# MingXiangL/SPE

Hardware: AMD Instinct MI355X
Metric: images/sec (whole node) at 3x800x1333 bs=2/GPU (higher is better)
Workload: dtype bf16/fp16 operands, fp32 accumulate; 1 GPU; TSCAM_cait_S24 (C=384, depth 24, 8 heads) + 0-layer encoder + 6-layer conditional-DETR decoder x2 stages, 100 queries, COCO heads (91), 2x3x800x1333 per GPU (N=4150 tokens), fwd + SetCriterion + SetCriterionRefine + bwd + grad all-reduce + clip + AdamW; global_batch=2, parallelism=dp1

## Files before the change

### include/spe_hip.h

```cpp
#ifndef SPE_HIP_H
#define SPE_HIP_H
#include <stddef.h>
#include <stdint.h>

#ifdef __cplusplus
extern "C" {
#endif

typedef struct ihipStream_t* spe_stream_t;

int spe_abi_version(void);

int spe_set_reduce_workspace(void* ws, size_t bytes, spe_stream_t stream);
int spe_reduce_defer_ranges(const void* const* ptrs, const size_t* bytes, int n);
int spe_reduce_defer_arena(void* arena, size_t bytes);
int spe_reduce_flush(spe_stream_t stream);
int spe_reduce_pending(void);

int spe_gemm_f32(const float* A, const float* B, float* C, const float* bias, float* C2,
                 int M, int N, int K, long lda, long ldb, long ldc, int transA, int transB,
                 int batch0, int batch1, long sA0, long sA1, long sB0, long sB1, long sC0, long sC1,
                 float alpha, int act, int splitk, int precision, spe_stream_t stream);

int spe_gemm_ex(const void* A, int a_bf16, const float* B, float* C, const float* bias, float* C2,
// ... 117 lines not shown
                          float* mean, float* rstd, long R, int C, float eps, float p, uint64_t seed, uint64_t offset,
                          spe_stream_t stream);
int spe_layernorm_res_bwd(const float* dy, const float* dy2, const float* sum, const float* gamma, const float* mean, const float* rstd,
                          float* ds, float* dz, float* dgamma, float* dbeta, long R, int C, float p, uint64_t seed,
                          uint64_t offset, spe_stream_t stream);

int spe_dropout(const float* x, float* y, long n, float p, uint64_t seed, uint64_t offset, spe_stream_t stream);

int spe_patchify(const float* img, float* cols, int B, int Cin, int Hi, int Wi, int P, spe_stream_t stream);

int spe_rowdot(const float* x, const float* y, float* D, int B, int L, int H, int dh, spe_stream_t stream);

int spe_add_rows(const float* a, const float* b, float* out, long n, long period, spe_stream_t stream);

int spe_bicubic(const float* src, float* dst, int gh, int gw, int h, int w, int C, int backward, spe_stream_t stream);

int spe_matcher_cost(const float* logits, const float* boxes, const int* tgt_ids, const float* tgt_boxes,
                     const int* toff, int total_targets, float* cost, int* err, int L, int B, int Q, int Kc,
                     float w_class, float w_bbox, float w_giou, spe_stream_t stream);

int spe_hungarian(const float* cost, const int* toff, long* srow, long* gidx, int* lidx, int* err, int L, int B, int Q,
                  spe_stream_t stream);
int spe_jitter_pick(const float* box, const float* scale, float* out, int M, int ncand, int ratio, spe_stream_t stream);

int spe_focal_loss(const float* logits, const int* tclass, const float* roww, float* grad, float* loss,
                   int* argmax, int L, long rows_per_l, int Kc, float alpha, float gamma, spe_stream_t stream);

int spe_box_loss(const float* pred_boxes, const long* srow, const float* tbox, const float* w, const int* lidx,
                 float* sums, float* g_l1, float* g_giou, long n, int L, spe_stream_t stream);
int spe_box_loss_bwd(const long* srow, const int* lidx, const float* g_l1, const float* g_giou, const float* c1,
                     const float* c2, float* dpred, long n, spe_stream_t stream);

int spe_kv_frags(const void* ym16, long ldm, const void* yp16, long ldp, void* Kf, void* V16, void* K16, void* Vf,
                 int L, int B, int S, int H, int dh, spe_stream_t stream);
int spe_kv_grad_scatter(const float* dk, const float* dv, void* dYm, long ldm, void* dYp, long ldp, int layer, int B, int S,
                        int H, int dh, spe_stream_t stream);
int spe_colsum_bf16_blocks(const void* x, long ld, long R, int nblk, int blkC, float* const* outs, int accumulate, spe_stream_t stream);

int spe_mha_plan(int B, int H, int Lq, int Lk, int* nch);
int spe_mha_fwd(const void* Qf, const void* Kf, const void* V16, const void* mask, float* Opart, float* ML, float* O,
                float* LSE, void* keepbits, int B, int H, int Lq, int Lk, int dk, int dv, int nch, float p_drop,
                uint64_t seed, uint64_t offset, spe_stream_t stream);
int spe_mha_bwd(const void* Qf, const void* Kf, const void* Vf, const void* dOf, const void* K16, const void* Q16,
                const void* dO16, const void* mask, const float* LSE, const float* D, const void* keepbits, float* dq,
                float* dq_ws, float* dk, float* dv, int B, int H, int Lq, int Lk, int dk_dim, int dv_dim, int nch, float scale,
                float p_drop, spe_stream_t stream);

int spe_pos_sine(const void* mask_u8, const float* dim_t, float* out, int B, int h, int w, int npf, float scale,
                 float eps, int normalize, spe_stream_t stream);

int spe_pos_learned_fwd(const float* col, const float* row, float* out, int B, int h, int w, int npf, spe_stream_t stream);
int spe_pos_learned_bwd(const float* g, float* d_col, float* d_row, int B, int h, int w, int npf, spe_stream_t stream);

int spe_nms_sorted(const float* boxes, const long* labels, const int* counts, unsigned char* keep, int nimg, int nmax,
                   float iou_threshold, spe_stream_t stream);

int spe_detect(const float* logits, const float* boxes, const float* sizes, int B, int Q, int Kc, int k, float iou_threshold,
               int do_nms, float* out_logit, long* out_label, float* out_box, int* out_query, int* out_count, spe_stream_t stream);

int spe_cam_prepare(const float* cams, int M, int h, int w, int rows, int cols, float cam_thr, float* minmax,
                    void* out, spe_stream_t stream);
int spe_cam_contour_boxes(const void* img, int rows, int cols, float area_ratio, int* boxes, int max_boxes, int* nboxes);
int spe_cam_boxes_device_workspace(int M, int rows, int cols, size_t* bytes);
int spe_cam_boxes_device(const void* img, int M, int rows, int cols, float area_ratio, void* workspace, size_t workspace_bytes,
                         int* boxes, int* nboxes, int max_boxes, spe_stream_t stream);

int spe_voc_match(const float* det_boxes, const float* det_scores, const long* det_labels, const int* det_off,
                  const double* gt_boxes, const long* gt_labels, const unsigned char* gt_difficult, const int* gt_off,
                  int nimg, int num_classes, int max_det, int max_gt, double ovthresh, double score_scale, double coord_scale,
                  unsigned char* flags, double* scores_out, int* npos, int* nimgs, int* hits, spe_stream_t stream);
int spe_voc_ap(const unsigned char* flags, const int* seg_off, const int* npos, int num_classes, double* ap07, double* ap_area,
               double* rec, double* prec, spe_stream_t stream);

int spe_coco_match(const float* det_boxes, const long* det_cats, const int* det_off, const double* gt_boxes, const long* gt_cats,
                   const unsigned char* gt_iscrowd, const double* gt_area, const int* gt_off, const double* iou_thrs,
                   const double* area_rng, int nimg, int num_cats, int max_det, int max_gt, int top, int* rank, unsigned* words,
                   int* npig, spe_stream_t stream);
int spe_coco_accumulate(const unsigned* words, const int* rank, const float* det_scores, const int* seg_off, const int* npig,
                        const int* max_dets, const double* rec_thrs, int num_cats, int num_rec, int num_max_dets, double* precision,
                        double* recall, double* scores, spe_stream_t stream);

int spe_resample_plan(long* desc_host, int n, long* totals);
int spe_resample_tables(const long* desc_host, const long* desc_dev, int n, int* tables, spe_stream_t stream);
int spe_resample_h(const long* desc_host, const long* desc_dev, int n, const int* tables, unsigned char* tmp, spe_stream_t stream);
int spe_resample_v(const long* desc_host, const long* desc_dev, int n, const int* tables, const unsigned char* tmp, const float* lut,
                   float* out, unsigned char* mask, int Hmax, int Wmax, spe_stream_t stream);

int spe_ledger_state_bytes(int K, int E, size_t* bytes);
int spe_ledger_record(const float* vals, const float* weights, const unsigned char* mask, const double* extras_host, int K, int E,
                      void* state, size_t state_bytes, float* total, spe_stream_t stream);
int spe_ledger_total_bwd(const float* g, const float* weights, const unsigned char* mask, int K, float* dvals, spe_stream_t stream);
int spe_ledger_summary(void* state, size_t state_bytes, int K, int E, const int* windows_host, const int* windows_dev,
                       const float* ring_override, const int* order, double* out, spe_stream_t stream);

int spe_sqnorm_partials(const float* g, long n, float* partials, int nblocks, spe_stream_t stream);
int spe_adamw_flat(float* p, float* g, float* m, float* v, long n, const long* seg_end, const float* seg_lr,
                   const float* seg_wd, int nseg, float beta1, float beta2, float eps, float bias_c1, float bias_c2,
                   const float* partials, int npartials, float max_norm, int write_grad, float grad_scale,
                   spe_stream_t stream);

int spe_accum_flat(float* dst, const float* a, const float* b, long n, spe_stream_t stream);

int spe_occupy(int nwg, long micros, float* buf, long buf_floats, spe_stream_t stream);

#ifdef __cplusplus
}
// ... 3 lines not shown
```

### spe_amd/build.py

```python
import glob
import hashlib
import os
import subprocess
import sys
from concurrent.futures import ThreadPoolExecutor

HERE = os.path.dirname(os.path.abspath(__file__))
CSRC = os.path.join(HERE, "csrc")
OBJ = os.path.join(HERE, "build")
LIB = os.path.join(HERE, "libspe_hip.so")
COMM_LIB = os.path.join(HERE, "libspe_comm.so")
STAMP = os.path.join(HERE, "libspe_hip.srchash")
FLAGS = ["--offload-arch=gfx950", "-O3", "-std=c++17", "-fPIC"]
EXTRA_FLAGS = {"attn_flash_bwd.hip": ["-mllvm", "-amdgpu-mfma-vgpr-form=1"],
               "voc_eval.hip": ["-ffp-contract=off"],
               "coco_eval.hip": ["-ffp-contract=off"],
               "img_resample.hip": ["-ffp-contract=off"],
               "step_ledger.hip": ["-ffp-contract=off"],
               "detect.hip": ["-ffp-contract=off"]}


def flags_for(src):
    return FLAGS + EXTRA_FLAGS.get(os.path.basename(src), [])


def sources():
    return sorted(glob.glob(os.path.join(CSRC, "*.hip")))


def _headers():
    return sorted(glob.glob(os.path.join(CSRC, "*.h")))


def _hash(files, extra=b""):
    h = hashlib.sha256(extra)
    for f in files:
        h.update(os.path.basename(f).encode())
        with open(f, "rb") as fh:
            h.update(fh.read())
    return h.hexdigest()


def _comm_sources():
    return sorted(glob.glob(os.path.join(CSRC, "comm", "*.hip"))) + [os.path.join(os.path.dirname(HERE), "include", "spe_comm.h")]


def source_hash():
    return _hash(sources() + _headers() + _comm_sources())


def needs_build():
    if not (os.path.exists(LIB) and os.path.exists(STAMP)):
        return True
    with open(STAMP) as fh:
        return fh.read().strip() != source_hash()


def _compile(src, hipcc, verbose):
    name = os.path.splitext(os.path.basename(src))[0]
    obj, tag = os.path.join(OBJ, name + ".o"), os.path.join(OBJ, name + ".hash")
    want = _hash([src] + _headers(), " ".join(flags_for(src)).encode())
    if os.path.exists(obj) and os.path.exists(tag) and open(tag).read().strip() == want:
        return obj
    cmd = [hipcc] + flags_for(src) + ["-c", src, "-o", obj + ".tmp"]
    if verbose:
        print(" ".join(cmd), file=sys.stderr, flush=True)
    subprocess.run(cmd, check=True, cwd=CSRC)
    os.replace(obj + ".tmp", obj)
    with open(tag, "w") as fh:
        fh.write(want + "\n")
    return obj

# ... 37 lines not shown
```

### spe_amd/kernels.py

```python
import ctypes
import os

import torch

from . import lib

_PRECISION = 2
import functools as _functools
import threading as _threading

_TLS = _threading.local()


def _in_bwd():
    return getattr(_TLS, "in_bwd", False)


def backward_scope(fn):
    @_functools.wraps(fn)
    def wrapped(ctx, *grads):
        prev, _TLS.in_bwd = _in_bwd(), True
        if _DEFER_FLATS is not None and not _FLUSH_QUEUED[0]:
            _FLUSH_QUEUED[0] = True
            try:
# ... 1406 lines not shown
    M, rows, cols = t.shape
    out = torch.empty((M * (1 + 4 * max_boxes),), device=t.device, dtype=torch.int32)
    if M:
        nbytes = cam_boxes_workspace_bytes(M, rows, cols)
        ws = torch.empty((nbytes // 4,), device=t.device, dtype=torch.int32)
        _call("spe_cam_boxes_device", _p(t), M, rows, cols, float(area_ratio), _p(ws), nbytes, _p(out[M:]), _p(out), max_boxes, _st())
    return out


def cam_boxes_device(imgs_u8_device, area_ratio, max_boxes=256):
    M = imgs_u8_device.shape[0]
    out = cam_boxes_device_packed(imgs_u8_device, area_ratio, max_boxes)
    return out[M:].view(M, max_boxes, 4), out[:M]


def pos_sine(mask_bool, dim_t, npf, scale, eps, normalize):
    B, h, w = mask_bool.shape
    m8 = mask_bool.to(torch.uint8).contiguous()
    out = torch.empty((B, h, w, 2 * npf), device=mask_bool.device, dtype=torch.float32)
    _call("spe_pos_sine", _p(m8), _p(dim_t), _p(out), B, h, w, npf, float(scale), float(eps), int(bool(normalize)), _st())
    return out


POS_TABLE_ROWS = 50


def pos_learned_fwd(col, row, B, h, w):
    _chk(col, row)
    npf = col.shape[1]
    if col.shape != (POS_TABLE_ROWS, npf) or row.shape != col.shape or not (col.is_contiguous() and row.is_contiguous()):
        raise ValueError(f"pos_learned_fwd: two contiguous [{POS_TABLE_ROWS}, npf] tables expected, got {tuple(col.shape)} and {tuple(row.shape)}")
    out = torch.empty((B, h, w, 2 * npf), device=col.device, dtype=torch.float32)
    _call("spe_pos_learned_fwd", _p(col), _p(row), _p(out), B, h, w, npf, _st())
    return out


def pos_learned_bwd(g, B, h, w, npf, need_col=True, need_row=True, dcol_out=None, drow_out=None):
    _chk(g, dcol_out, drow_out)
    if g.numel() != B * h * w * 2 * npf or not g.is_contiguous():
        raise ValueError(f"pos_learned_bwd: a contiguous gradient of {B} x {h} x {w} x {2 * npf} elements expected, got {tuple(g.shape)}")
    outs = []
    for need, o in ((need_col, dcol_out), (need_row, drow_out)):
        if not need:
            o = None
        elif o is None:
            o = torch.empty((POS_TABLE_ROWS, npf), device=g.device, dtype=torch.float32)
        elif o.shape != (POS_TABLE_ROWS, npf) or not o.is_contiguous():
            raise ValueError(f"pos_learned_bwd: destination {tuple(o.shape)} is not a contiguous [{POS_TABLE_ROWS}, {npf}]")
        outs.append(o)
    _call("spe_pos_learned_bwd", _p(g), _p(outs[0]), _p(outs[1]), B, h, w, npf, _st())
    return outs[0], outs[1]


MAX_DET = 4096
VOC_MAX_DET = COCO_MAX_DET = MAX_DET


def _check_typed(name, pairs):
    for t, dt in pairs:
        if not t.is_cuda:
            raise lib.SpeLibraryError("spe_amd kernels run on the GPU only (got a CPU tensor); there is no CPU fallback")
        if t.dtype != dt or not t.is_contiguous():
            raise TypeError(f"{name}: expected a contiguous {dt} tensor, got {t.dtype}")


VOC_MAX_GT = 1024


def voc_match(det_boxes, det_scores, det_labels, det_off, gt_boxes, gt_labels, gt_difficult, gt_off, max_det, max_gt,
              ovthresh, score_scale, coord_scale, npos, nimgs, hits):
    _check_typed("voc_match", ((det_boxes, torch.float32), (det_scores, torch.float32), (det_labels, torch.int64), (det_off, torch.int32),
                               (gt_boxes, torch.float64), (gt_labels, torch.int64), (gt_difficult, torch.uint8), (gt_off, torch.int32),
                               (npos, torch.int32), (nimgs, torch.int32), (hits, torch.int32)))
    nd, C, nimg = det_scores.numel(), npos.numel(), det_off.numel() - 1
    if gt_off.numel() != nimg + 1 or nimgs.numel() != C or hits.numel() != C or det_boxes.numel() != nd * 4 or \
            det_labels.numel() != nd or gt_boxes.numel() != gt_labels.numel() * 4 or gt_difficult.numel() != gt_labels.numel():
        raise ValueError("voc_match: inconsistent shapes")
    flags = torch.empty((nd,), device=det_scores.device, dtype=torch.uint8)
    scores = torch.empty((nd,), device=det_scores.device, dtype=torch.float64)
    _call("spe_voc_match", _p(det_boxes), _p(det_scores), _p(det_labels), _p(det_off), _p(gt_boxes), _p(gt_labels), _p(gt_difficult),
          _p(gt_off), nimg, C, int(max_det), int(max_gt), float(ovthresh), float(score_scale), float(coord_scale), _p(flags),
          _p(scores), _p(npos), _p(nimgs), _p(hits), _st())
    return flags, scores


def voc_ap(flags, seg_off, npos, want_curve=False):
    _check_typed("voc_ap", ((flags, torch.uint8), (seg_off, torch.int32), (npos, torch.int32)))
    C = npos.numel()
    if seg_off.numel() != C + 1:
        raise ValueError("voc_ap: seg_off must hold num_classes + 1 offsets")
    ap = torch.empty((2, C), device=flags.device, dtype=torch.float64)
    rec = torch.empty((flags.numel(),), device=flags.device, dtype=torch.float64) if want_curve else None
    prec = torch.empty_like(rec) if want_curve else None
    _call("spe_voc_ap", _p(flags), _p(seg_off), _p(npos), C, _p(ap[0]), _p(ap[1]), _p(rec), _p(prec), _st())
    return ap[0], ap[1], rec, prec


COCO_MAX_GT = 512
COCO_T, COCO_A = 10, 4
COCO_MAX_REC = 128


def coco_match(det_boxes, det_cats, det_off, gt_boxes, gt_cats, gt_iscrowd, gt_area, gt_off, iou_thrs, area_rng, max_det, max_gt,
               top, npig):
    _check_typed("coco_match", ((det_boxes, torch.float32), (det_cats, torch.int64), (det_off, torch.int32), (gt_boxes, torch.float64),
                                (gt_cats, torch.int64), (gt_iscrowd, torch.uint8), (gt_area, torch.float64), (gt_off, torch.int32),
# ... 114 lines not shown
```

### spe_amd/models/conditional_detr.py

```python
import math

import torch
import torch.nn.functional as F
from torch import nn
from torch.autograd import Function

from .. import kernels as K
from ..util import box_ops
from ..util.misc import (NestedTensor, get_world_size, host_to_device, inverse_sigmoid, is_dist_avail_and_initialized,
                         nested_tensor_from_tensor_list)
from .cait_backbone import build_backbone
from .layers import MLP, Linear
from .matcher import build_matcher
from .transformer import build_transformer


class ConditionalDETR_Refine(nn.Module):

    def __init__(self, backbone, transformer, num_classes, num_queries, aux_loss=False, num_refines=1, drloc=False):
        super().__init__()
        self.num_queries = num_queries
        self.num_refines = num_refines
        self.transformer = transformer
        hidden_dim = transformer.d_model
        self.class_embed = nn.ModuleList([Linear(hidden_dim, num_classes) for _ in range(num_refines + 1)])
        self.bbox_embed = nn.ModuleList([MLP(hidden_dim, hidden_dim, 4, 3) for _ in range(num_refines + 1)])
        self.query_embed = nn.Embedding(num_queries, hidden_dim)
        self.queries_embed_refine = nn.ModuleList([nn.Embedding(num_queries, hidden_dim) for _ in range(num_refines)])
        self.backbone = backbone
        self.aux_loss = aux_loss
        bias_value = -math.log((1 - 0.01) / 0.01)
        for ce in self.class_embed:
            ce.bias.data = torch.ones(num_classes) * bias_value
        for be in self.bbox_embed:
            nn.init.constant_(be.layers[-1].weight.data, 0)
            nn.init.constant_(be.layers[-1].bias.data, 0)

    def forward(self, samples: NestedTensor):
        if isinstance(samples, (list, torch.Tensor)):
            samples = nested_tensor_from_tensor_list(samples)
        _, _, H, W = samples.decompose()[0].size()
        ps = self.backbone[0].body.patch_size
        self.transformer.H, self.transformer.W = H // ps, W // ps
        features, pos = self.backbone(samples)
        src, mask = features["x_patch"].decompose()
        assert mask is not None
        Hs, references = self.transformer(src, mask, self.query_embed.weight, pos[-1],
                                          queries_embed_refine=self.queries_embed_refine)
        out = {}
        for r in range(self.num_refines + 1):
            hs = Hs[r]
            ref_before = inverse_sigmoid(references[r])
            tmp = self.bbox_embed[r](hs)
            tmp = torch.cat([tmp[..., :2] + ref_before, tmp[..., 2:]], dim=-1)
            outputs_coord = tmp.sigmoid()
            outputs_class = self.class_embed[r](hs)
            o = {"pred_logits": outputs_class[-1], "pred_boxes": outputs_coord[-1], **features}
            if self.aux_loss:
                o["aux_outputs"] = [{"pred_logits": a, "pred_boxes": b}
                                    for a, b in zip(outputs_class[:-1], outputs_coord[:-1])]
            out[r] = o
        return out


class _FocalLoss(Function):

    @staticmethod
    def forward(ctx, logits, tclass, roww, alpha, gamma, num_boxes):
        loss, grad, amax = K.focal_loss(logits, tclass, roww, alpha, gamma)
        ctx.save_for_backward(grad)
        ctx.nb = num_boxes
        ctx.mark_non_differentiable(amax)
        return loss / num_boxes, amax

    @staticmethod
    def backward(ctx, dloss, _):
        (grad,) = ctx.saved_tensors
        return grad * (dloss / ctx.nb).view(-1, 1, 1), None, None, None, None, None


class _BoxLoss(Function):

    @staticmethod
    def forward(ctx, pred_flat, srow, tbox, w, lidx, L, num_boxes):
        sums, g1, g2 = K.box_loss(pred_flat, srow, tbox, w, lidx, L)
        ctx.save_for_backward(srow, lidx, g1, g2)
        ctx.nb, ctx.shape = num_boxes, pred_flat.shape
        return sums / num_boxes

    @staticmethod
    def backward(ctx, d):
        srow, lidx, g1, g2 = ctx.saved_tensors
        d = (d / ctx.nb).contiguous()
        dpred = K.box_loss_bwd(srow, lidx, g1, g2, d[:, 0].contiguous(), d[:, 1].contiguous(), ctx.shape)
        return dpred, None, None, None, None, None, None


JITTER_KERNEL = True


def jitter_targets(targets, ratio, jitter):
    out = [dict(t) for t in targets]
    counts = [t["boxes"].shape[0] for t in out]
    if sum(counts) > 0:
        box = torch.cat([t["boxes"] for t in out if t["boxes"].shape[0] > 0])
        M = box.shape[0]
        scale = torch.empty((M, 1000, 4), dtype=box.dtype, device=box.device).uniform_(1 - jitter, 1 + jitter)
        if JITTER_KERNEL and box.is_cuda and box.dtype == torch.float32:
# ... 251 lines not shown
```

### spe_amd/models/transformer.py

```python
import copy
import math

import torch
from torch import nn

from .. import ops
from .attention import MultiheadAttention
from .layers import MLP, Dropout, LayerNorm, Linear


def gen_sineembed_for_position(pos_tensor, d_model=256):
    n_steps = d_model // 2
    scale = 2 * math.pi
    dim_t = torch.arange(n_steps, dtype=torch.float32, device=pos_tensor.device)
    dim_t = 10000 ** (2 * torch.div(dim_t, 2, rounding_mode="floor") / 128)
    pos_x = pos_tensor[..., 0, None] * scale / dim_t
    pos_y = pos_tensor[..., 1, None] * scale / dim_t
    pos_x = torch.stack((pos_x[..., 0::2].sin(), pos_x[..., 1::2].cos()), dim=-1).flatten(-2)
    pos_y = torch.stack((pos_y[..., 0::2].sin(), pos_y[..., 1::2].cos()), dim=-1).flatten(-2)
    return torch.cat((pos_y, pos_x), dim=-1)


class PackedSelfAttention(nn.Module):

    def __init__(self, embed_dim, num_heads, dropout=0.0):
        super().__init__()
        self.embed_dim, self.num_heads, self.dropout = embed_dim, num_heads, float(dropout)
        self.in_proj_weight = nn.Parameter(torch.empty(3 * embed_dim, embed_dim))
        self.in_proj_bias = nn.Parameter(torch.zeros(3 * embed_dim))
        self.out_proj = Linear(embed_dim, embed_dim)
        nn.init.xavier_uniform_(self.in_proj_weight)
        nn.init.constant_(self.out_proj.bias, 0.0)

    def forward(self, qk_in, v_in, key_padding_mask):
        B, S, d = qk_in.shape
        H = self.num_heads
        qk = ops.linear(qk_in, self.in_proj_weight[:2 * d], self.in_proj_bias[:2 * d]).view(B, S, 2, H, d // H)
        v = ops.linear(v_in, self.in_proj_weight[2 * d:], self.in_proj_bias[2 * d:]).view(B, S, H, d // H)
        o, _ = ops.attention(qk[:, :, 0], qk[:, :, 1], v, key_padding_mask, float(d // H) ** -0.5,
                             self.dropout if self.training else 0.0)
        return self.out_proj(o)


class TransformerEncoderLayer(nn.Module):
    def __init__(self, d_model, nhead, dim_feedforward=2048, dropout=0.1, activation="relu", normalize_before=False):
        super().__init__()
        if normalize_before:
            raise NotImplementedError("pre-norm is not reachable in the reference (transformer.py:461-462)")
        self.self_attn = PackedSelfAttention(d_model, nhead, dropout=dropout)
        self.linear1 = Linear(d_model, dim_feedforward)
        self.dropout = Dropout(dropout)
        self.linear2 = Linear(dim_feedforward, d_model)
        self.norm1 = LayerNorm(d_model)
        self.norm2 = LayerNorm(d_model)
        self.dropout1 = Dropout(dropout)
        self.dropout2 = Dropout(dropout)

    def forward(self, src, src_key_padding_mask=None, pos=None):
        qk = src if pos is None else ops.add(src, pos)
        src2 = self.self_attn(qk, src, src_key_padding_mask)
        src, src_skip = self.norm1.residual2(src, src2, self.dropout1)
        src2 = self.linear2(self.dropout(self.linear1(src, ops.ACT_RELU)))
        return self.norm2.residual(src_skip, src2, self.dropout2)

# ... 16 lines not shown
class TransformerDecoderLayer(nn.Module):
    def __init__(self, d_model, nhead, dim_feedforward=2048, dropout=0.1, activation="relu", normalize_before=False):
        super().__init__()
        self.sa_qcontent_proj = Linear(d_model, d_model)
        self.sa_qpos_proj = Linear(d_model, d_model)
        self.sa_kcontent_proj = Linear(d_model, d_model)
        self.sa_kpos_proj = Linear(d_model, d_model)
        self.sa_v_proj = Linear(d_model, d_model)
        self.self_attn = MultiheadAttention(d_model, nhead, dropout=dropout, vdim=d_model)
        self.ca_qcontent_proj = Linear(d_model, d_model)
        self.ca_qpos_proj = Linear(d_model, d_model)
        self.ca_kcontent_proj = Linear(d_model, d_model)
        self.ca_kpos_proj = Linear(d_model, d_model)
        self.ca_v_proj = Linear(d_model, d_model)
        self.ca_qpos_sine_proj = Linear(d_model, d_model)
        self.cross_attn = MultiheadAttention(d_model * 2, nhead, dropout=dropout, vdim=d_model)
        self.nhead = nhead
        self.linear1 = Linear(d_model, dim_feedforward)
        self.dropout = Dropout(dropout)
        self.linear2 = Linear(dim_feedforward, d_model)
        self.norm1 = LayerNorm(d_model)
        self.norm2 = LayerNorm(d_model)
        self.norm3 = LayerNorm(d_model)
        self.dropout1 = Dropout(dropout)
        self.dropout2 = Dropout(dropout)
        self.dropout3 = Dropout(dropout)

    def memory_side(self, memory, pos, is_first):
        B, S, d = memory.shape
        H, dh = self.nhead, d // self.nhead
        k_content = self.ca_kcontent_proj(memory)
        v = self.ca_v_proj(memory)
        k_pos = self.ca_kpos_proj(pos)
        k = ops.add(k_content, k_pos) if is_first else k_content
        k = torch.cat([k.view(B, S, H, dh), k_pos.view(B, S, H, dh)], dim=3)
        return k.view(B, S, 2 * d), v

    def forward(self, tgt, mem_kv, memory_key_padding_mask, query_pos, query_sine_embed, is_first, n_stages=1, qp=None):
        B, RQ, d = tgt.shape
        H, dh = self.nhead, d // self.nhead
        Q = RQ // n_stages
        q_pos, k_pos, ca_pos = qp if qp is not None else (self.sa_qpos_proj(query_pos), self.sa_kpos_proj(query_pos), None)
        content = (self.sa_qcontent_proj, self.sa_kcontent_proj, self.sa_v_proj)
        if ops.group_linear_ok(tgt, content):
            q, k, v = ops.group_linear(tgt, content, adds=(q_pos, k_pos, None))
        else:
            q, k, v = (m(tgt) for m in content)
            q = q + q_pos
            k = k + k_pos
        sa = lambda t: t.view(B * n_stages, Q, d)
        tgt2 = self.self_attn(sa(q), sa(k), sa(v))[0].view(B, RQ, d)
        tgt, tgt_skip = self.norm1.residual2(tgt, tgt2, self.dropout1)
        q = self.ca_qcontent_proj(tgt)
        if is_first:
            q = q + (ca_pos if ca_pos is not None else self.ca_qpos_proj(query_pos))
        qs = self.ca_qpos_sine_proj(query_sine_embed)
        if isinstance(mem_kv[0], ops.MemoryKV):
            holder, tok, layer_id = mem_kv
            if is_first:
                qs = qs + q
            q = torch.cat([q.view(B, RQ, H, dh), qs.view(B, RQ, H, dh)], dim=3)
            ca = self.cross_attn
            o = ops.cross_attention_kv(q, tok, holder, layer_id, memory_key_padding_mask, float(ca.head_dim) ** -0.5,
                                       ca.dropout if ca.training else 0.0)
            tgt2 = ca.out_proj(o)
        else:
            q = torch.cat([q.view(B, RQ, H, dh), qs.view(B, RQ, H, dh)], dim=3).view(B, RQ, 2 * d)
            k, v = mem_kv
            tgt2 = self.cross_attn(q, k, v, key_padding_mask=memory_key_padding_mask)[0]
        tgt, tgt_skip = self.norm2.residual2(tgt_skip, tgt2, self.dropout2)
        tgt2 = self.linear2(self.dropout(self.linear1(tgt, ops.ACT_RELU)))
        return self.norm3.residual(tgt_skip, tgt2, self.dropout3)


class TransformerDecoder(nn.Module):
    def __init__(self, decoder_layer, num_layers, norm=None, return_intermediate=False, d_model=256):
        super().__init__()
        self.layers = _get_clones(decoder_layer, num_layers)
        self.num_layers = num_layers
        self.norm = norm
        self.return_intermediate = return_intermediate
        self.d_model = d_model
        self.query_scale = MLP(d_model, d_model, d_model, 2)
        self.ref_point_head = MLP(d_model, d_model, 2, 2)
        for layer_id in range(num_layers - 1):
            self.layers[layer_id + 1].ca_qpos_proj = None

    def _memory_side_all(self, memory, pos, mem_cache):
        mem_w = [m for layer in self.layers for m in (layer.ca_kcontent_proj, layer.ca_v_proj)]
        pos_w = [layer.ca_kpos_proj for layer in self.layers]
        Wm, bm = [m.weight for m in mem_w], [m.bias for m in mem_w]
        Wp, bp = [m.weight for m in pos_w], [m.bias for m in pos_w]
        if not (memory.is_cuda and ops.multi_linear_ok(memory, Wm, bm) and ops.multi_linear_ok(pos, Wp, bp)):
            return
        B, S, d = memory.shape
        H, dh = self.layers[0].nhead, d // self.layers[0].nhead
        if ops.memory_side_kv_ok(memory, Wm, Wp, H):
            holder, toks = ops.memory_side_kv(memory, pos, H, Wm, Wp, bm, bp)
            for l in range(len(self.layers)):
                mem_cache[l] = (holder, toks[l], l)
            return
        ym = ops.multi_linear(memory, Wm, bm)
        yp = ops.multi_linear(pos, Wp, bp)
        for l in range(len(self.layers)):
            kc, v, kp = ym[2 * l], ym[2 * l + 1], yp[l]
            k = kc + kp if l == 0 else kc
            k = torch.cat([k.view(B, S, H, dh), kp.view(B, S, H, dh)], dim=3)
            mem_cache[l] = (k.view(B, S, 2 * d), v)

    def _query_pos_all(self, query_pos):
        mods = [m for layer in self.layers for m in (layer.sa_qpos_proj, layer.sa_kpos_proj)] + [self.layers[0].ca_qpos_proj]
        if not ops.group_linear_ok(query_pos, mods[:2]):
            return None
        outs = []
        for i in range(0, len(mods), 16):
            chunk = mods[i:i + 16]
            outs += list(ops.group_linear(query_pos, chunk)) if len(chunk) > 1 else [chunk[0](query_pos)]
        return [(outs[2 * l], outs[2 * l + 1], outs[-1] if l == 0 else None) for l in range(len(self.layers))]

    def forward(self, tgt, memory, memory_key_padding_mask, pos, query_pos, mem_cache=None, n_stages=1):
        mem_cache = {} if mem_cache is None else mem_cache
        output = tgt
        reference_points = self.ref_point_head(query_pos).sigmoid()
        intermediate = []
        sine0 = gen_sineembed_for_position(reference_points[..., :2], self.d_model)
        if not mem_cache:
            self._memory_side_all(memory, pos, mem_cache)
        qp_all = self._query_pos_all(query_pos)
        for layer_id, layer in enumerate(self.layers):
            if layer_id not in mem_cache:
                mem_cache[layer_id] = layer.memory_side(memory, pos, layer_id == 0)
            sine = sine0
            if layer_id > 0:
                sine = sine0 * self.query_scale(output)
            output = layer(output, mem_cache[layer_id], memory_key_padding_mask, query_pos, sine, layer_id == 0,
                           n_stages=n_stages, qp=None if qp_all is None else qp_all[layer_id])
            intermediate.append(self.norm(output))
        return torch.stack(intermediate), reference_points


class Transformer(nn.Module):
    def __init__(self, d_model=512, nhead=8, num_queries=300, num_encoder_layers=6, num_decoder_layers=6,
                 dim_feedforward=2048, dropout=0.1, activation="relu", normalize_before=False,
                 return_intermediate_dec=False, args=None, num_refines=1, drloc=False):
        super().__init__()
        enc_layer = TransformerEncoderLayer(d_model, nhead, dim_feedforward, dropout, activation, normalize_before)
        self.encoder = TransformerEncoder(enc_layer, num_encoder_layers, None)
        dec_layer = TransformerDecoderLayer(d_model, nhead, dim_feedforward, dropout, activation, normalize_before)
        self.decoder = TransformerDecoder(dec_layer, num_decoder_layers, LayerNorm(d_model),
                                          return_intermediate=return_intermediate_dec, d_model=d_model)
        self.H = self.W = None
        self._reset_parameters()
        self.d_model, self.nhead = d_model, nhead
        self.dec_layers, self.num_queries, self.num_refines = num_decoder_layers, num_queries, num_refines

    def _reset_parameters(self):
        for p in self.parameters():
            if p.dim() > 1:
                nn.init.xavier_uniform_(p)

    def forward(self, src, mask, query_embed, pos_embed, queries_embed_refine=None):
        B = src.shape[0]
        memory = src.flatten(2).transpose(1, 2).contiguous()
        pos = pos_embed.flatten(2).transpose(1, 2).contiguous()
        mask = mask.flatten(1)
        memory = self.encoder(memory, src_key_padding_mask=mask, pos=pos)
        queries = [query_embed] + [qe.weight for qe in (queries_embed_refine or [])]
        R, Q = len(queries), query_embed.shape[0]
        query_pos = torch.stack(queries).reshape(1, R * Q, -1).expand(B, -1, -1).contiguous()
        h, r = self.decoder(torch.zeros_like(query_pos), memory, mask, pos, query_pos, n_stages=R)
        hs = [h[:, :, i * Q:(i + 1) * Q] for i in range(R)]
        refs = [r[:, i * Q:(i + 1) * Q] for i in range(R)]
        return hs, refs


def _get_clones(module, n):
    return nn.ModuleList([copy.deepcopy(module) for _ in range(n)])


def build_transformer(args):
    return Transformer(d_model=args.hidden_dim, dropout=args.dropout, nhead=args.nheads, num_queries=args.num_queries,
                       dim_feedforward=args.dim_feedforward, num_encoder_layers=args.enc_layers,
                       num_decoder_layers=args.dec_layers, normalize_before=args.pre_norm, return_intermediate_dec=True)
```

### spe_amd/ops.py

```python
import os

import torch
from torch.autograd import Function

from . import kernels as K

ACT_NONE, ACT_RELU, ACT_GELU = 0, 1, 2


class _Linear(Function):

    @staticmethod
    @K.forward_scope
    def forward(ctx, x, W, b, act):
        shp = x.shape
        x2 = x.reshape(-1, shp[-1])
        if not x2.is_contiguous():
            x2 = x2.contiguous()
        Wc = W if W.is_contiguous() else W.contiguous()
        y, pre, xsave = K.linear_fwd(x2, Wc, b, act, want_pre=(act == ACT_GELU), save_for_dw=ctx.needs_input_grad[1], src=x)
        aux = pre if act == ACT_GELU else (y if act == ACT_RELU else None)
        ctx.act = act
        ctx.has_bias = b is not None
        ctx.params = (W, b)
# ... 1044 lines not shown
    def backward(ctx, dy):
        return dy, dy


def add(a, b):
    assert a.shape == b.shape
    return _Add.apply(a, b)


class _BicubicGrid(Function):

    @staticmethod
    @K.forward_scope
    def forward(ctx, pe, gh, gw, h, w):
        ctx.g = (gh, gw, h, w)
        return K.bicubic(pe[0].contiguous(), gh, gw, h, w).unsqueeze(0)

    @staticmethod
    @K.backward_scope
    def backward(ctx, dy):
        gh, gw, h, w = ctx.g
        return K.bicubic(dy[0].contiguous(), gh, gw, h, w, backward=True).unsqueeze(0), None, None, None, None


def bicubic_grid(pe, gh, gw, h, w):
    return _BicubicGrid.apply(pe, gh, gw, h, w)


class _PosLearned(Function):

    @staticmethod
    @K.forward_scope
    def forward(ctx, col, row, B, h, w):
        if any(ctx.needs_input_grad[:2]):
            ctx.g = (B, h, w, col.shape[1])
            ctx.params = (col, row)
        return K.pos_learned_fwd(col, row, B, h, w)

    @staticmethod
    @K.backward_scope
    def backward(ctx, dy):
        B, h, w, npf = ctx.g
        need_c, need_r = ctx.needs_input_grad[:2]
        colp, rowp = ctx.params
        dc, dr = K.pos_learned_bwd(dy.contiguous(), B, h, w, npf, need_c, need_r,
                                   K.grad_buffer(colp) if need_c else None, K.grad_buffer(rowp) if need_r else None)
        return dc, dr, None, None, None


def pos_learned(col, row, B, h, w):
    return _PosLearned.apply(col, row, int(B), int(h), int(w))


class _LedgerTotal(Function):

    @staticmethod
    def forward(ctx, vals, weights, mask, extras, state):
        ctx.save_for_backward(weights, mask)
        if vals.is_cuda:
            return K.ledger_record(vals, weights, mask, extras, state)
        from . import steplog
        return steplog.record_host(vals, weights, mask, extras, state)

    @staticmethod
    def backward(ctx, g):
        weights, mask = ctx.saved_tensors
        if g.is_cuda:
            return K.ledger_total_bwd(g.contiguous(), weights, mask), None, None, None, None
        return torch.where(mask != 0, weights * g, torch.zeros_like(weights)), None, None, None, None


def ledger_total(vals, weights, mask, extras, state):
    return _LedgerTotal.apply(vals, weights, mask, tuple(extras), state)
```

Baseline: 42.42 images/sec.

## Fuse decoder query construction, sine embedding, scaling and box head into custom kernels

Adds custom HIP forward and backward kernels for four pieces of the conditional-DETR decoder: the sine position embedding, the cross-attention query build (add, carry and per-head concat), the elementwise query-scale multiply, and the box head (inverse-sigmoid of the reference plus sigmoid). Each one replaces a chain of small PyTorch elementwise, cat and view ops, in both forward and autograd backward, to cut kernel launches and intermediate tensors. These shapes are small (100 queries, 6 layers, 2 stages), so the saving is mostly launch overhead. The cost is custom backward maths, such as the clamp handling in inverse-sigmoid, which has to match autograd exactly.

```diff
diff --git a/include/spe_hip.h b/include/spe_hip.h
--- a/include/spe_hip.h
+++ b/include/spe_hip.h
@@ -193,6 +193,17 @@
 int spe_pos_learned_fwd(const float* col, const float* row, float* out, int B, int h, int w, int npf, spe_stream_t stream);
 int spe_pos_learned_bwd(const float* g, float* d_col, float* d_row, int B, int h, int w, int npf, spe_stream_t stream);
 
+int spe_sine_embed_fwd(const float* ref, const float* dim_t, float* out, long rows, int n, spe_stream_t stream);
+int spe_sine_embed_bwd(const float* dout, const float* ref, const float* dim_t, float* dref, long rows, int n, spe_stream_t stream);
+int spe_query_build_fwd(const float* qc, long ldc, const float* pos, long ldp, const float* qs, long lds, float* q, long rows, int H,
+                        int dh, int carry, spe_stream_t stream);
+int spe_query_build_bwd(const float* dq, float* dqc, float* dqs, long rows, int H, int dh, int carry, spe_stream_t stream);
+int spe_mul_fwd(const float* a, const float* b, float* y, long n, spe_stream_t stream);
+int spe_mul_bwd(const float* dy, const float* a, const float* b, float* da, float* db, long n, spe_stream_t stream);
+int spe_box_head_fwd(const float* tmp, const float* ref, long ref_bs, float* coord, int L, int B, int Q, spe_stream_t stream);
+int spe_box_head_bwd(const float* dcoord, const float* coord, const float* ref, long ref_bs, float* dtmp, float* dref, int L, int B, int Q,
+                     spe_stream_t stream);
+
 int spe_nms_sorted(const float* boxes, const long* labels, const int* counts, unsigned char* keep, int nimg, int nmax,
                    float iou_threshold, spe_stream_t stream);
 
diff --git a/spe_amd/build.py b/spe_amd/build.py
--- a/spe_amd/build.py
+++ b/spe_amd/build.py
@@ -17,7 +17,8 @@
                "coco_eval.hip": ["-ffp-contract=off"],
                "img_resample.hip": ["-ffp-contract=off"],
                "step_ledger.hip": ["-ffp-contract=off"],
-               "detect.hip": ["-ffp-contract=off"]}
+               "detect.hip": ["-ffp-contract=off"],
+               "decoder_query.hip": ["-ffp-contract=off"]}
 
 
 def flags_for(src):
diff --git a/spe_amd/csrc/decoder_query.hip b/spe_amd/csrc/decoder_query.hip
--- /dev/null
+++ b/spe_amd/csrc/decoder_query.hip
@@ -0,0 +1,235 @@
+#include "common.h"
+
+template <int V> struct QVec;
+template <> struct QVec<4> {
+    typedef float4 T;
+    static __device__ __forceinline__ T add(T a, T b) { return spe_add4(a, b); }
+    static __device__ __forceinline__ T mul(T a, T b) { return spe_mul4(a, b); }
+};
+template <> struct QVec<1> {
+    typedef float T;
+    static __device__ __forceinline__ T add(T a, T b) { return a + b; }
+    static __device__ __forceinline__ T mul(T a, T b) { return a * b; }
+};
+
+static bool dq_aligned16(const void* a, const void* b = nullptr, const void* c = nullptr, const void* d = nullptr, const void* e = nullptr) {
+    return ((reinterpret_cast<uintptr_t>(a) | reinterpret_cast<uintptr_t>(b) | reinterpret_cast<uintptr_t>(c) | reinterpret_cast<uintptr_t>(d) |
+             reinterpret_cast<uintptr_t>(e)) & 15) == 0;
+}
+static unsigned dq_blocks(long total) {
+    long nb = (total + 255) / 256;
+    return (unsigned)(nb < 1 ? 1 : (nb > 4096 ? 4096 : nb));
+}
+
+#define SINE_SCALE 6.283185307179586f
+
+__global__ __launch_bounds__(256) void sine_embed_fwd_kernel(const float* __restrict__ ref, const float* __restrict__ dim_t,
+                                                             float* __restrict__ out, long rows, int n) {
+    const long total = rows * 2 * n;
+    for (long i = (long)blockIdx.x * 256 + threadIdx.x; i < total; i += (long)gridDim.x * 256) {
+        const int c = (int)(i % (2 * n));
+        const long row = i / (2 * n);
+        const int half = c >= n, j = c - half * n;
+        const float v = ref[row * 2 + (1 - half)] * SINE_SCALE / dim_t[j];
+        out[i] = (j & 1) ? cosf(v) : sinf(v);
+    }
+}
+
+__global__ __launch_bounds__(128) void sine_embed_bwd_kernel(const float* __restrict__ dout, const float* __restrict__ ref,
+                                                             const float* __restrict__ dim_t, float* __restrict__ dref, int n) {
+    const long row = blockIdx.x;
+    const int half = threadIdx.x >> 6, lane = threadIdx.x & 63;
+    const float x = ref[row * 2 + (1 - half)];
+    const float* g = dout + row * 2 * n + (long)half * n;
+    float acc = 0.f;
+    for (int j = lane; j < n; j += 64) {
+        const float t = dim_t[j];
+        const float v = x * SINE_SCALE / t;
+        const float dv = (j & 1) ? g[j] * -sinf(v) : g[j] * cosf(v);
+        acc += dv / t * SINE_SCALE;
+    }
+    acc = spe_wave_sum(acc);
+    if (lane == 0) dref[row * 2 + (1 - half)] = acc;
+}
+
+template <int V>
+__global__ __launch_bounds__(256) void query_build_fwd_kernel(const float* __restrict__ qc, long ldc, const float* __restrict__ pos, long ldp,
+                                                              const float* __restrict__ qs, long lds, float* __restrict__ q, long rows,
+                                                              int H, int dh, int carry) {
+    typedef typename QVec<V>::T vec_t;
+    const int CW = H * dh / V, hw = dh / V;
+    const long total = rows * CW;
+    for (long i = (long)blockIdx.x * 256 + threadIdx.x; i < total; i += (long)gridDim.x * 256) {
+        const int cu = (int)(i % CW);
+        const long row = i / CW;
+        const int h = cu / hw, e = cu - h * hw;
+        vec_t a = *reinterpret_cast<const vec_t*>(qc + row * ldc + (long)cu * V);
+        if (pos) a = QVec<V>::add(a, *reinterpret_cast<const vec_t*>(pos + row * ldp + (long)cu * V));
+        vec_t s = *reinterpret_cast<const vec_t*>(qs + row * lds + (long)cu * V);
+        if (carry) s = QVec<V>::add(s, a);
+        float* o = q + (row * H + h) * 2L * dh + (long)e * V;
+        *reinterpret_cast<vec_t*>(o) = a;
+        *reinterpret_cast<vec_t*>(o + dh) = s;
+    }
+}
+
+template <int V>
+__global__ __launch_bounds__(256) void query_build_bwd_kernel(const float* __restrict__ dq, float* __restrict__ dqc, float* __restrict__ dqs,
+                                                              long rows, int H, int dh, int carry) {
+    typedef typename QVec<V>::T vec_t;
+    const int CW = H * dh / V, hw = dh / V;
+    const long total = rows * CW;
+    for (long i = (long)blockIdx.x * 256 + threadIdx.x; i < total; i += (long)gridDim.x * 256) {
+        const int cu = (int)(i % CW);
+        const long row = i / CW;
+        const int h = cu / hw, e = cu - h * hw;
+        const float* g = dq + (row * H + h) * 2L * dh + (long)e * V;
+        vec_t a = *reinterpret_cast<const vec_t*>(g);
+        const vec_t s = *reinterpret_cast<const vec_t*>(g + dh);
+        if (carry) a = QVec<V>::add(a, s);
+        reinterpret_cast<vec_t*>(dqc)[i] = a;
+        reinterpret_cast<vec_t*>(dqs)[i] = s;
+    }
+}
+
+template <int V>
+__global__ __launch_bounds__(256) void mul_fwd_kernel(const float* __restrict__ a, const float* __restrict__ b, float* __restrict__ y, long nv) {
+    typedef typename QVec<V>::T vec_t;
+    for (long i = (long)blockIdx.x * 256 + threadIdx.x; i < nv; i += (long)gridDim.x * 256)
+        reinterpret_cast<vec_t*>(y)[i] = QVec<V>::mul(reinterpret_cast<const vec_t*>(a)[i], reinterpret_cast<const vec_t*>(b)[i]);
+}
+template <int V>
+__global__ __launch_bounds__(256) void mul_bwd_kernel(const float* __restrict__ dy, const float* __restrict__ a, const float* __restrict__ b,
+                                                      float* __restrict__ da, float* __restrict__ db, long nv) {
+    typedef typename QVec<V>::T vec_t;
+    for (long i = (long)blockIdx.x * 256 + threadIdx.x; i < nv; i += (long)gridDim.x * 256) {
+        const vec_t g = reinterpret_cast<const vec_t*>(dy)[i];
+        reinterpret_cast<vec_t*>(da)[i] = QVec<V>::mul(g, reinterpret_cast<const vec_t*>(b)[i]);
+        reinterpret_cast<vec_t*>(db)[i] = QVec<V>::mul(g, reinterpret_cast<const vec_t*>(a)[i]);
+    }
+}
+
+#define INV_SIGMOID_EPS 1e-5f
+__device__ __forceinline__ float dq_clamp_min(float x, float lo) { return x < lo ? lo : x; }
+__device__ __forceinline__ float dq_clamp_max(float x, float hi) { return x > hi ? hi : x; }
+__device__ __forceinline__ float dq_sigmoid(float x) { return 1.0f / (1.0f + expf(-x)); }
+
+__global__ __launch_bounds__(256) void box_head_fwd_kernel(const float* __restrict__ tmp, const float* __restrict__ ref, long ref_bs,
+                                                           float* __restrict__ coord, int L, int B, int Q) {
+    const long total = (long)L * B * Q;
+    for (long i = (long)blockIdx.x * 256 + threadIdx.x; i < total; i += (long)gridDim.x * 256) {
+        const int q = (int)(i % Q), b = (int)((i / Q) % B);
+        const float* r = ref + b * ref_bs + (long)q * 2;
+        float inv[2];
+#pragma unroll
+        for (int c = 0; c < 2; ++c) {
+            const float x = dq_clamp_max(dq_clamp_min(r[c], 0.f), 1.f);
+            inv[c] = logf(dq_clamp_min(x, INV_SIGMOID_EPS) / dq_clamp_min(1.0f - x, INV_SIGMOID_EPS));
+        }
+        const float4 t = reinterpret_cast<const float4*>(tmp)[i];
+        reinterpret_cast<float4*>(coord)[i] = make_float4(dq_sigmoid(t.x + inv[0]), dq_sigmoid(t.y + inv[1]), dq_sigmoid(t.z), dq_sigmoid(t.w));
+    }
+}
+
+__global__ __launch_bounds__(256) void box_head_bwd_kernel(const float* __restrict__ dcoord, const float* __restrict__ coord,
+                                                           const float* __restrict__ ref, long ref_bs, float* __restrict__ dtmp,
+                                                           float* __restrict__ dref, int L, int B, int Q) {
+    const long BQ = (long)B * Q;
+    for (long i = (long)blockIdx.x * 256 + threadIdx.x; i < BQ; i += (long)gridDim.x * 256) {
+        float gs[2] = {0.f, 0.f};
+        for (int l = 0; l < L; ++l) {
+            const float4 g = reinterpret_cast<const float4*>(dcoord)[l * BQ + i], s = reinterpret_cast<const float4*>(coord)[l * BQ + i];
+            const float4 d = make_float4(g.x * (1.0f - s.x) * s.x, g.y * (1.0f - s.y) * s.y, g.z * (1.0f - s.z) * s.z, g.w * (1.0f - s.w) * s.w);
+            reinterpret_cast<float4*>(dtmp)[l * BQ + i] = d;
+            gs[0] = l ? gs[0] + d.x : d.x;
+            gs[1] = l ? gs[1] + d.y : d.y;
+        }
+        if (!dref) continue;
+        const int q = (int)(i % Q), b = (int)(i / Q);
+        const float* r = ref + b * ref_bs + (long)q * 2;
+#pragma unroll
+        for (int c = 0; c < 2; ++c) {
+            const float r0 = r[c];
+            const float x = dq_clamp_max(dq_clamp_min(r0, 0.f), 1.f);
+            const float u = 1.0f - x;
+            const float num = dq_clamp_min(x, INV_SIGMOID_EPS), den = dq_clamp_min(u, INV_SIGMOID_EPS);
+            const float gr = gs[c] / (num / den);
+            const float gnum = gr / den, gden = -gr * ((num / den) / den);
+            const float gx_num = x >= INV_SIGMOID_EPS ? gnum : 0.f;
+            const float gu = u >= INV_SIGMOID_EPS ? gden : 0.f;
+            const float gx = gx_num + -gu;
+            dref[i * 2 + c] = (r0 >= 0.f && r0 <= 1.f) ? gx : 0.f;
+        }
+    }
+}
+
+extern "C" int spe_sine_embed_fwd(const float* ref, const float* dim_t, float* out, long rows, int n, hipStream_t st) {
+    if (rows < 1 || n < 2 || (n & 1)) return -2;
+    hipLaunchKernelGGL(sine_embed_fwd_kernel, dim3(dq_blocks(rows * 2 * n)), dim3(256), 0, st, ref, dim_t, out, rows, n);
+    SPE_CHECK_LAUNCH();
+    return 0;
+}
+
+extern "C" int spe_sine_embed_bwd(const float* dout, const float* ref, const float* dim_t, float* dref, long rows, int n, hipStream_t st) {
+    if (rows < 1 || rows > 0x7fffffffL || n < 2 || (n & 1)) return -2;
+    hipLaunchKernelGGL(sine_embed_bwd_kernel, dim3((unsigned)rows), dim3(128), 0, st, dout, ref, dim_t, dref, n);
+    SPE_CHECK_LAUNCH();
+    return 0;
+}
+
+extern "C" int spe_query_build_fwd(const float* qc, long ldc, const float* pos, long ldp, const float* qs, long lds, float* q, long rows, int H,
+                                   int dh, int carry, hipStream_t st) {
+    const long d = (long)H * dh;
+    if (rows < 1 || H < 1 || dh < 1 || ldc < d || lds < d || (pos && ldp < d)) return -2;
+    const bool v4 = (dh & 3) == 0 && ((ldc | lds | (pos ? ldp : 0)) & 3) == 0 && dq_aligned16(qc, pos, qs, q);
+    const dim3 grid(dq_blocks(rows * (d / (v4 ? 4 : 1))));
+    if (v4) hipLaunchKernelGGL(query_build_fwd_kernel<4>, grid, dim3(256), 0, st, qc, ldc, pos, ldp, qs, lds, q, rows, H, dh, carry);
+    else hipLaunchKernelGGL(query_build_fwd_kernel<1>, grid, dim3(256), 0, st, qc, ldc, pos, ldp, qs, lds, q, rows, H, dh, carry);
+    SPE_CHECK_LAUNCH();
+    return 0;
+}
+
+extern "C" int spe_query_build_bwd(const float* dq, float* dqc, float* dqs, long rows, int H, int dh, int carry, hipStream_t st) {
+    if (rows < 1 || H < 1 || dh < 1) return -2;
+    const bool v4 = (dh & 3) == 0 && dq_aligned16(dq, dqc, dqs);
+    const dim3 grid(dq_blocks(rows * ((long)H * dh / (v4 ? 4 : 1))));
+    if (v4) hipLaunchKernelGGL(query_build_bwd_kernel<4>, grid, dim3(256), 0, st, dq, dqc, dqs, rows, H, dh, carry);
+    else hipLaunchKernelGGL(query_build_bwd_kernel<1>, grid, dim3(256), 0, st, dq, dqc, dqs, rows, H, dh, carry);
+    SPE_CHECK_LAUNCH();
+    return 0;
+}
+
+extern "C" int spe_mul_fwd(const float* a, const float* b, float* y, long n, hipStream_t st) {
+    if (n < 1) return -2;
+    const bool v4 = (n & 3) == 0 && dq_aligned16(a, b, y);
+    const long nv = v4 ? n / 4 : n;
+    if (v4) hipLaunchKernelGGL(mul_fwd_kernel<4>, dim3(dq_blocks(nv)), dim3(256), 0, st, a, b, y, nv);
+    else hipLaunchKernelGGL(mul_fwd_kernel<1>, dim3(dq_blocks(nv)), dim3(256), 0, st, a, b, y, nv);
+    SPE_CHECK_LAUNCH();
+    return 0;
+}
+
+extern "C" int spe_mul_bwd(const float* dy, const float* a, const float* b, float* da, float* db, long n, hipStream_t st) {
+    if (n < 1) return -2;
+    const bool v4 = (n & 3) == 0 && dq_aligned16(dy, a, b, da, db);
+    const long nv = v4 ? n / 4 : n;
+    if (v4) hipLaunchKernelGGL(mul_bwd_kernel<4>, dim3(dq_blocks(nv)), dim3(256), 0, st, dy, a, b, da, db, nv);
+    else hipLaunchKernelGGL(mul_bwd_kernel<1>, dim3(dq_blocks(nv)), dim3(256), 0, st, dy, a, b, da, db, nv);
+    SPE_CHECK_LAUNCH();
+    return 0;
+}
+
+extern "C" int spe_box_head_fwd(const float* tmp, const float* ref, long ref_bs, float* coord, int L, int B, int Q, hipStream_t st) {
+    if (L < 1 || B < 1 || Q < 1 || ref_bs < 2L * Q || !dq_aligned16(tmp, coord)) return -2;
+    hipLaunchKernelGGL(box_head_fwd_kernel, dim3(dq_blocks((long)L * B * Q)), dim3(256), 0, st, tmp, ref, ref_bs, coord, L, B, Q);
+    SPE_CHECK_LAUNCH();
+    return 0;
+}
+
+extern "C" int spe_box_head_bwd(const float* dcoord, const float* coord, const float* ref, long ref_bs, float* dtmp, float* dref, int L, int B,
+                                int Q, hipStream_t st) {
+    if (L < 1 || B < 1 || Q < 1 || ref_bs < 2L * Q || !dq_aligned16(dcoord, coord, dtmp)) return -2;
+    hipLaunchKernelGGL(box_head_bwd_kernel, dim3(dq_blocks((long)B * Q)), dim3(256), 0, st, dcoord, coord, ref, ref_bs, dtmp, dref, L, B, Q);
+    SPE_CHECK_LAUNCH();
+    return 0;
+}
diff --git a/spe_amd/kernels.py b/spe_amd/kernels.py
--- a/spe_amd/kernels.py
+++ b/spe_amd/kernels.py
@@ -1482,6 +1482,117 @@
     return outs[0], outs[1]
 
 
+_SINE_DIM_T = {}
+
+
+def sine_dim_t(n, device):
+    key = (device.index if device.index is not None else torch.cuda.current_device(), int(n))
+    t = _SINE_DIM_T.get(key)
+    if t is None:
+        with torch.no_grad():
+            j = torch.arange(n, dtype=torch.float32, device=device)
+            t = _SINE_DIM_T[key] = (10000 ** (2 * torch.div(j, 2, rounding_mode="floor") / 128)).contiguous()
+    return t
+
+
+def _rows_ok(name, t, cols):
+    if t.dim() != 2 or t.shape[1] != cols or t.stride(1) != 1:
+        raise ValueError(f"{name}: a [rows, {cols}] tensor with unit column stride expected, got shape {tuple(t.shape)} strides {t.stride()}")
+    return t.stride(0) if t.shape[0] > 1 else max(t.stride(0), cols)
+
+
+def sine_embed_fwd(ref, dim_t):
+    _chk(ref, dim_t)
+    rows, n = ref.shape[0], dim_t.numel()
+    if ref.shape != (rows, 2) or not ref.is_contiguous():
+        raise ValueError(f"sine_embed_fwd: a contiguous [rows, 2] tensor expected, got {tuple(ref.shape)}")
+    out = torch.empty((rows, 2 * n), device=ref.device, dtype=torch.float32)
+    _call("spe_sine_embed_fwd", _p(ref), _p(dim_t), _p(out), rows, n, _st())
+    return out
+
+
+def sine_embed_bwd(dout, ref, dim_t):
+    _chk(dout, ref, dim_t)
+    rows, n = ref.shape[0], dim_t.numel()
+    if dout.shape != (rows, 2 * n) or not dout.is_contiguous():
+        raise ValueError(f"sine_embed_bwd: a contiguous [{rows}, {2 * n}] gradient expected, got {tuple(dout.shape)}")
+    dref = torch.empty((rows, 2), device=ref.device, dtype=torch.float32)
+    _call("spe_sine_embed_bwd", _p(dout), _p(ref), _p(dim_t), _p(dref), rows, n, _st())
+    return dref
+
+
+def query_build_fwd(qc, pos, qs, H, carry):
+    _chk(qc, pos, qs)
+    rows, d = qc.shape
+    if d % H:
+        raise ValueError(f"query_build_fwd: width {d} does not split into {H} heads")
+    ldc, lds = _rows_ok("query_build_fwd", qc, d), _rows_ok("query_build_fwd", qs, d)
+    ldp = 0 if pos is None else _rows_ok("query_build_fwd", pos, d)
+    if qs.shape[0] != rows or (pos is not None and pos.shape[0] != rows):
+        raise ValueError("query_build_fwd: the operands differ in their row count")
+    q = torch.empty((rows, H, 2 * (d // H)), device=qc.device, dtype=torch.float32)
+    _call("spe_query_build_fwd", _p(qc), ldc, _p(pos), ldp, _p(qs), lds, _p(q), rows, H, d // H, int(bool(carry)), _st())
+    return q
+
+
+def query_build_bwd(dq, H, carry):
+    _chk(dq)
+    rows, dh = dq.shape[0], dq.shape[2] // 2
+    if dq.dim() != 3 or dq.shape[1] != H or dq.shape[2] != 2 * dh or not dq.is_contiguous():
+        raise ValueError(f"query_build_bwd: a contiguous [rows, {H}, 2 * dh] gradient expected, got {tuple(dq.shape)}")
+    dqc = torch.empty((rows, H * dh), device=dq.device, dtype=torch.float32)
+    dqs = torch.empty_like(dqc)
+    _call("spe_query_build_bwd", _p(dq), _p(dqc), _p(dqs), rows, H, dh, int(bool(carry)), _st())
+    return dqc, dqs
+
+
+def mul_fwd(a, b):
+    _chk(a, b)
+    if a.shape != b.shape or not (a.is_contiguous() and b.is_contiguous()):
+        raise ValueError(f"mul_fwd: two contiguous tensors of one shape expected, got {tuple(a.shape)} and {tuple(b.shape)}")
+    y = torch.empty_like(a)
+    _call("spe_mul_fwd", _p(a), _p(b), _p(y), a.numel(), _st())
+    return y
+
+
+def mul_bwd(dy, a, b):
+    _chk(dy, a, b)
+    if dy.shape != a.shape or a.shape != b.shape or not (dy.is_contiguous() and a.is_contiguous() and b.is_contiguous()):
+        raise ValueError(f"mul_bwd: three contiguous tensors of one shape expected, got {tuple(dy.shape)}, {tuple(a.shape)}, {tuple(b.shape)}")
+    da, db = torch.empty_like(a), torch.empty_like(a)
+    _call("spe_mul_bwd", _p(dy), _p(a), _p(b), _p(da), _p(db), a.numel(), _st())
+    return da, db
+
+
+def _box_head_ref(name, ref, B, Q):
+    if ref.shape != (B, Q, 2) or ref.stride(2) != 1 or ref.stride(1) != 2:
+        raise ValueError(f"{name}: reference points [{B}, {Q}, 2] with dense rows expected, got shape {tuple(ref.shape)} strides {ref.stride()}")
+    return max(ref.stride(0), 2 * Q)
+
+
+def box_head_fwd(tmp, ref):
+    _chk(tmp, ref)
+    if tmp.dim() != 4 or tmp.shape[3] != 4 or not tmp.is_contiguous():
+        raise ValueError(f"box_head_fwd: a contiguous [L, B, Q, 4] tensor expected, got {tuple(tmp.shape)}")
+    L, B, Q, _ = tmp.shape
+    ref_bs = _box_head_ref("box_head_fwd", ref, B, Q)
+    coord = torch.empty_like(tmp)
+    _call("spe_box_head_fwd", _p(tmp), _p(ref), ref_bs, _p(coord), L, B, Q, _st())
+    return coord
+
+
+def box_head_bwd(dcoord, coord, ref, need_dref=True):
+    _chk(dcoord, coord, ref)
+    if dcoord.shape != coord.shape or not (dcoord.is_contiguous() and coord.is_contiguous()):
+        raise ValueError(f"box_head_bwd: a contiguous gradient of shape {tuple(coord.shape)} expected, got {tuple(dcoord.shape)}")
+    L, B, Q, _ = coord.shape
+    ref_bs = _box_head_ref("box_head_bwd", ref, B, Q)
+    dtmp = torch.empty_like(coord)
+    dref = torch.empty((B, Q, 2), device=coord.device, dtype=torch.float32) if need_dref else None
+    _call("spe_box_head_bwd", _p(dcoord), _p(coord), _p(ref), ref_bs, _p(dtmp), _p(dref), L, B, Q, _st())
+    return dtmp, dref
+
+
 MAX_DET = 4096
 VOC_MAX_DET = COCO_MAX_DET = MAX_DET
 
diff --git a/spe_amd/models/conditional_detr.py b/spe_amd/models/conditional_detr.py
--- a/spe_amd/models/conditional_detr.py
+++ b/spe_amd/models/conditional_detr.py
@@ -6,6 +6,7 @@
 from torch.autograd import Function
 
 from .. import kernels as K
+from .. import ops
 from ..util import box_ops
 from ..util.misc import (NestedTensor, get_world_size, host_to_device, inverse_sigmoid, is_dist_avail_and_initialized,
                          nested_tensor_from_tensor_list)
@@ -50,10 +51,13 @@
         out = {}
         for r in range(self.num_refines + 1):
             hs = Hs[r]
-            ref_before = inverse_sigmoid(references[r])
             tmp = self.bbox_embed[r](hs)
-            tmp = torch.cat([tmp[..., :2] + ref_before, tmp[..., 2:]], dim=-1)
-            outputs_coord = tmp.sigmoid()
+            if ops.box_head_ok(tmp, references[r]):
+                outputs_coord = ops.box_head(tmp, references[r])
+            else:
+                ref_before = inverse_sigmoid(references[r])
+                tmp = torch.cat([tmp[..., :2] + ref_before, tmp[..., 2:]], dim=-1)
+                outputs_coord = tmp.sigmoid()
             outputs_class = self.class_embed[r](hs)
             o = {"pred_logits": outputs_class[-1], "pred_boxes": outputs_coord[-1], **features}
             if self.aux_loss:
diff --git a/spe_amd/models/transformer.py b/spe_amd/models/transformer.py
--- a/spe_amd/models/transformer.py
+++ b/spe_amd/models/transformer.py
@@ -10,6 +10,8 @@
 
 
 def gen_sineembed_for_position(pos_tensor, d_model=256):
+    if ops.sine_embed_ok(pos_tensor, d_model):
+        return ops.sine_embed(pos_tensor, d_model)
     n_steps = d_model // 2
     scale = 2 * math.pi
     dim_t = torch.arange(n_steps, dtype=torch.float32, device=pos_tensor.device)
@@ -132,21 +134,27 @@
         tgt2 = self.self_attn(sa(q), sa(k), sa(v))[0].view(B, RQ, d)
         tgt, tgt_skip = self.norm1.residual2(tgt, tgt2, self.dropout1)
         q = self.ca_qcontent_proj(tgt)
-        if is_first:
-            q = q + (ca_pos if ca_pos is not None else self.ca_qpos_proj(query_pos))
+        q_add = (ca_pos if ca_pos is not None else self.ca_qpos_proj(query_pos)) if is_first else None
         qs = self.ca_qpos_sine_proj(query_sine_embed)
-        if isinstance(mem_kv[0], ops.MemoryKV):
-            holder, tok, layer_id = mem_kv
+        memkv = isinstance(mem_kv[0], ops.MemoryKV)
+        carry = is_first and memkv
+        if ops.query_build_ok(q, q_add, qs):
+            q = ops.query_build(q, q_add, qs, H, carry)
+        else:
             if is_first:
+                q = q + q_add
+            if carry:
                 qs = qs + q
             q = torch.cat([q.view(B, RQ, H, dh), qs.view(B, RQ, H, dh)], dim=3)
+        if memkv:
+            holder, tok, layer_id = mem_kv
             ca = self.cross_attn
             o = ops.cross_attention_kv(q, tok, holder, layer_id, memory_key_padding_mask, float(ca.head_dim) ** -0.5,
                                        ca.dropout if ca.training else 0.0)
             tgt2 = ca.out_proj(o)
         else:
-            q = torch.cat([q.view(B, RQ, H, dh), qs.view(B, RQ, H, dh)], dim=3).view(B, RQ, 2 * d)
             k, v = mem_kv
+            q = q.view(B, RQ, 2 * d)
             tgt2 = self.cross_attn(q, k, v, key_padding_mask=memory_key_padding_mask)[0]
         tgt, tgt_skip = self.norm2.residual2(tgt_skip, tgt2, self.dropout2)
         tgt2 = self.linear2(self.dropout(self.linear1(tgt, ops.ACT_RELU)))
@@ -212,7 +220,8 @@
                 mem_cache[layer_id] = layer.memory_side(memory, pos, layer_id == 0)
             sine = sine0
             if layer_id > 0:
-                sine = sine0 * self.query_scale(output)
+                scale = self.query_scale(output)
+                sine = ops.mul(sine0, scale) if ops.mul_ok(sine0, scale) else sine0 * scale
             output = layer(output, mem_cache[layer_id], memory_key_padding_mask, query_pos, sine, layer_id == 0,
                            n_stages=n_stages, qp=None if qp_all is None else qp_all[layer_id])
             intermediate.append(self.norm(output))
diff --git a/spe_amd/ops.py b/spe_amd/ops.py
--- a/spe_amd/ops.py
+++ b/spe_amd/ops.py
@@ -1120,6 +1120,115 @@
     return _PosLearned.apply(col, row, int(B), int(h), int(w))
 
 
+QUERY_KERNELS = True
+
+
+def _plain(*ts):
+    return QUERY_KERNELS and all(t.is_cuda and t.dtype == torch.float32 for t in ts if t is not None)
+
+
+class _SineEmbed(Function):
+
+    @staticmethod
+    @K.forward_scope
+    def forward(ctx, ref, n):
+        ref2 = ref.reshape(-1, 2)
+        dim_t = K.sine_dim_t(n, ref.device)
+        ctx.save_for_backward(ref2, dim_t)
+        return K.sine_embed_fwd(ref2, dim_t).view(*ref.shape[:-1], 2 * n)
+
+    @staticmethod
+    @K.backward_scope
+    def backward(ctx, dout):
+        ref2, dim_t = ctx.saved_tensors
+        dref = K.sine_embed_bwd(dout.reshape(ref2.shape[0], -1).contiguous(), ref2, dim_t)
+        return dref.view(*dout.shape[:-1], 2), None
+
+
+def sine_embed_ok(pos_tensor, d_model):
+    return _plain(pos_tensor) and pos_tensor.shape[-1] == 2 and pos_tensor.is_contiguous() and d_model % 4 == 0 and pos_tensor.numel() > 0
+
+
+def sine_embed(pos_tensor, d_model):
+    return _SineEmbed.apply(pos_tensor, d_model // 2)
+
+
+class _QueryBuild(Function):
+
+    @staticmethod
+    @K.forward_scope
+    def forward(ctx, qc, pos, qs, H, carry):
+        B, Lq, d = qc.shape
+        ctx.meta = (H, carry, qc.shape)
+        two = lambda t: None if t is None else t.reshape(B * Lq, d)
+        return K.query_build_fwd(two(qc), two(pos), two(qs), H, carry).view(B, Lq, H, 2 * (d // H))
+
+    @staticmethod
+    @K.backward_scope
+    def backward(ctx, dq):
+        H, carry, shp = ctx.meta
+        dqc, dqs = K.query_build_bwd(dq.contiguous().view(shp[0] * shp[1], H, -1), H, carry)
+        dqc, dqs = dqc.view(shp), dqs.view(shp)
+        return dqc, (dqc if ctx.needs_input_grad[1] else None), dqs, None, None
+
+
+def query_build_ok(qc, pos, qs):
+    rows = lambda t: t is None or (t.shape == qc.shape and t.is_contiguous())
+    return _plain(qc, pos, qs) and qc.dim() == 3 and qc.numel() > 0 and rows(qc) and rows(pos) and rows(qs)
+
+
+def query_build(qc, pos, qs, H, carry):
+    return _QueryBuild.apply(qc, pos, qs, int(H), bool(carry))
+
+
+class _Mul(Function):
+
+    @staticmethod
+    @K.forward_scope
+    def forward(ctx, a, b):
+        ctx.save_for_backward(a, b)
+        return K.mul_fwd(a, b)
+
+    @staticmethod
+    @K.backward_scope
+    def backward(ctx, dy):
+        a, b = ctx.saved_tensors
+        return K.mul_bwd(dy.contiguous(), a, b)
+
+
+def mul_ok(a, b):
+    return _plain(a, b) and a.shape == b.shape and a.is_contiguous() and b.is_contiguous() and a.numel() > 0
+
+
+def mul(a, b):
+    return _Mul.apply(a, b)
+
+
+class _BoxHead(Function):
+
+    @staticmethod
+    @K.forward_scope
+    def forward(ctx, tmp, ref):
+        coord = K.box_head_fwd(tmp, ref)
+        ctx.save_for_backward(coord, ref)
+        return coord
+
+    @staticmethod
+    @K.backward_scope
+    def backward(ctx, dcoord):
+        coord, ref = ctx.saved_tensors
+        return K.box_head_bwd(dcoord.contiguous(), coord, ref, ctx.needs_input_grad[1])
+
+
+def box_head_ok(tmp, ref):
+    return (_plain(tmp, ref) and tmp.dim() == 4 and tmp.shape[3] == 4 and tmp.is_contiguous() and tmp.numel() > 0 and tmp.data_ptr() % 16 == 0
+            and ref.shape == tmp.shape[1:3] + (2,) and ref.stride(2) == 1 and ref.stride(1) == 2)
+
+
+def box_head(tmp, ref):
+    return _BoxHead.apply(tmp, ref)
+
+
 class _LedgerTotal(Function):
 
     @staticmethod
```

Result: no change. 42.37 images/sec (-0.1%).
